# yingqichao/video-watermarking-forgery-detection

Measured on AMD Instinct MI355X. Metric: frames/sec training step (embed->JPEG->decode), 256x256, higher is better.
Workload: dtype bf16; 1 GPU; C2: HiDDeN GAN step enc(4x64)->Jpeg50->dec(7x64)+disc(3x64), L=30, 256x256, batch 16/GPU; not launched (results identical): the generator pass's dead discriminator weight gradients, the decoder's input gradient that Jpeg's zero-gradient rounding multiplies by 0 -- reference_state (--full) times the step with them; global_batch=16, parallelism=dp1

## Files before the change

video_watermarking_forgery_detection_amd/csrc/heads.hip:

```cpp
#include "wm_common.h"

namespace {

template <typename T, int COUT>
__global__ __launch_bounds__(256) void head_fwd_kernel(const T* __restrict__ y, int ldy, const float* __restrict__ scale,
                                                       const float* __restrict__ shift, const float* __restrict__ w,
                                                       const float* __restrict__ bias, float* __restrict__ out, size_t npix,
                                                       size_t hw, int Cin, int act, T* __restrict__ act16) {
    constexpr int VE = vec16<T>::N;
    const int VPP = Cin / VE, PPB = 256 / VPP;
    const int vv = threadIdx.x % VPP, ps = threadIdx.x / VPP;
    const int c0 = vv * VE;
    float sc[VE], sh[VE], wr[COUT][VE];
#pragma unroll
    for (int e = 0; e < VE; ++e) {
        sc[e] = scale ? scale[c0 + e] : 1.f;
        sh[e] = scale ? shift[c0 + e] : 0.f;
#pragma unroll
        for (int co = 0; co < COUT; ++co) wr[co][e] = w[co * Cin + c0 + e];
    }
    constexpr int UN = 4;
    for (size_t base = (size_t)blockIdx.x * PPB * UN; base < npix; base += (size_t)gridDim.x * PPB * UN) {
        vec16<T> yv[UN];
        bool valid[UN];
#pragma unroll
        for (int u = 0; u < UN; ++u) {
            const size_t p = base + (size_t)u * PPB + ps;
            valid[u] = p < npix;
            yv[u] = *reinterpret_cast<const vec16<T>*>(y + (valid[u] ? p : npix - 1) * ldy + c0);
        }
#pragma unroll
        for (int u = 0; u < UN; ++u) {
            const size_t p = base + (size_t)u * PPB + ps;
            float part[COUT];
#pragma unroll
            for (int co = 0; co < COUT; ++co) part[co] = 0.f;
#pragma unroll
            for (int e = 0; e < VE; ++e) {
                float a = sc[e] * yv[u].get(e) + sh[e];
                if (scale) a = fmaxf(a, 0.f);
#pragma unroll
                for (int co = 0; co < COUT; ++co) part[co] += wr[co][e] * a;
            }
            for (int o = VPP >> 1; o > 0; o >>= 1) {
#pragma unroll
                for (int co = 0; co < COUT; ++co) part[co] += __shfl_xor(part[co], o, 64);
            }
            if (valid[u]) {
                for (int oc = vv; oc < COUT; oc += VPP) {
                    float v = 0.f;
#pragma unroll
                    for (int co = 0; co < COUT; ++co) v = (oc == co) ? part[co] + bias[co] : v;
                    if (act == 1) v = 1.f / (1.f + __expf(-v));
                    const size_t b = p / hw, q = p - b * hw;
                    out[(b * COUT + oc) * hw + q] = v;
                }
            }
            if (act16 && valid[u]) {
                for (int pc = vv; pc < 16 / VE; pc += VPP) {
                    vec16<T> o;
#pragma unroll
                    for (int e = 0; e < VE; ++e) {
                        float val = 0.f;
#pragma unroll
                        for (int co = 0; co < COUT; ++co) val = (pc * VE + e == co) ? part[co] + bias[co] : val;
                        o.set(e, val);
                    }
                    *reinterpret_cast<vec16<T>*>(act16 + p * 16 + pc * VE) = o;
                }
            }
        }
    }
}

template <typename T, int COUT>
__global__ __launch_bounds__(256) void head_bwd_kernel(const T* __restrict__ y, int ldy, const float* __restrict__ scale,
                                                       const float* __restrict__ shift, const float* __restrict__ w,
                                                       const float* __restrict__ gout, T* __restrict__ g, int ldg,
                                                       float* __restrict__ partials, size_t npix, size_t hw, int Cin,
                                                       float* __restrict__ bn_partials) {
    constexpr int VE = vec16<T>::N;
    const int VPP = Cin / VE, PPB = 256 / VPP;
    const int vv = threadIdx.x % VPP, ps = threadIdx.x / VPP;
    const int c0 = vv * VE;
    float sc[VE], sh[VE], wr[COUT][VE], dw[COUT][VE], db[COUT];
#pragma unroll
    for (int e = 0; e < VE; ++e) {
        sc[e] = scale ? scale[c0 + e] : 1.f;
        sh[e] = scale ? shift[c0 + e] : 0.f;
#pragma unroll
        for (int co = 0; co < COUT; ++co) { wr[co][e] = w[co * Cin + c0 + e]; dw[co][e] = 0.f; }
    }
#pragma unroll
    for (int co = 0; co < COUT; ++co) db[co] = 0.f;
    float b1[VE], b2[VE];
#pragma unroll
    for (int e = 0; e < VE; ++e) { b1[e] = 0.f; b2[e] = 0.f; }
    for (size_t p = (size_t)blockIdx.x * PPB + ps; p < npix; p += (size_t)gridDim.x * PPB) {
        const size_t b = p / hw, q = p - b * hw;
        float go[COUT];
#pragma unroll
        for (int co = 0; co < COUT; ++co) go[co] = gout[(b * COUT + co) * hw + q];
        const vec16<T> yv = *reinterpret_cast<const vec16<T>*>(y + p * ldy + c0);
        vec16<T> gv;
#pragma unroll
        for (int e = 0; e < VE; ++e) {
            float a = sc[e] * yv.get(e) + sh[e];
            if (scale) a = fmaxf(a, 0.f);
            float gg = 0.f;
#pragma unroll
            for (int co = 0; co < COUT; ++co) { gg += go[co] * wr[co][e]; dw[co][e] += go[co] * a; }
            gv.set(e, gg);
            if (bn_partials) {
                const float gz = a > 0.f ? gv.get(e) : 0.f;
                b1[e] += gz;
                b2[e] = __builtin_fmaf(gz, yv.get(e), b2[e]);
            }
        }
        if (vv == 0) {
#pragma unroll
            for (int co = 0; co < COUT; ++co) db[co] += go[co];
        }
// ... 15 lines not shown
        float s = 0.f;
        for (int qq = 0; qq < PPB; ++qq) s += red[qq * VPP + v2][co * VE + e];
        prow[i] = s;
    }
    if (threadIdx.x < COUT) {
        float s = 0.f;
        for (int qq = 0; qq < PPB; ++qq) s += red[qq * VPP][COUT * VE + threadIdx.x];
        prow[COUT * Cin + threadIdx.x] = s;
    }
    if (bn_partials) {
        __syncthreads();
#pragma unroll
        for (int e = 0; e < VE; ++e) { red[threadIdx.x][e] = b1[e]; red[threadIdx.x][VE + e] = b2[e]; }
        __syncthreads();
        for (int i = threadIdx.x; i < 2 * Cin; i += 256) {
            const int which = i / Cin, c = i - which * Cin;
            const int v2 = c / VE, e = c - v2 * VE;
            float s = 0.f;
            for (int qq = 0; qq < PPB; ++qq) s += red[qq * VPP + v2][which * VE + e];
            bn_partials[((size_t)blockIdx.x * 2 + which) * Cin + c] = s;
        }
    }
}

bool cin_ok(int Cin, int dtype) {
    const int ve = dtype != WM_F32 ? 8 : 4;
    if (Cin <= 0 || Cin % ve) return false;
    const int vpp = Cin / ve;
    return vpp <= 64 && (vpp & (vpp - 1)) == 0;
}

inline int head_parts(size_t npix) {
    const size_t n = (npix + 511) / 512;
    return (int)(n < 1 ? 1 : (n > 1024 ? 1024 : n));
}

}

extern "C" int wm_conv1x1_head_fwd(const void* y, int ldy, const float* scale, const float* shift, const float* w,
                                   const float* bias, float* out, int B, size_t hw, int Cin, int Cout, int act, int dtype,
                                   void* stream) {
    return wm_conv1x1_head_fwd_act(y, ldy, scale, shift, w, bias, out, nullptr, B, hw, Cin, Cout, act, dtype, stream);
}

extern "C" int wm_conv1x1_head_fwd_act(const void* y, int ldy, const float* scale, const float* shift, const float* w,
                                       const float* bias, float* out, void* act16, int B, size_t hw, int Cin, int Cout, int act, int dtype,
                                       void* stream) {
    WM_REQUIRE(y && w && bias && out, WM_E_BADARG, "wm_conv1x1_head_fwd: null pointer");
    WM_REQUIRE(!act16 || (act == 0 && ((uintptr_t)act16 & 15) == 0), WM_E_BADARG, "wm_conv1x1_head_fwd_act: act16 goes with act == 0 and a 16-byte aligned pointer");
    WM_REQUIRE((scale == nullptr) == (shift == nullptr), WM_E_BADARG, "wm_conv1x1_head_fwd: scale/shift must come together");
    WM_REQUIRE(cin_ok(Cin, dtype), WM_E_SHAPE, "wm_conv1x1_head_fwd: unsupported Cin=%d", Cin);
    WM_REQUIRE(Cout == 1 || Cout == 3, WM_E_SHAPE, "wm_conv1x1_head_fwd: Cout must be 1 or 3 (got %d)", Cout);
    const size_t npix = (size_t)B * hw;
    const int grid = (int)((npix + 127) / 128 > 2048 ? 2048 : (npix + 127) / 128);
    hipStream_t s = (hipStream_t)stream;
    WM_DISPATCH_DTYPE(dtype, "wm_conv1x1_head_fwd",
        if (Cout == 3) hipLaunchKernelGGL((head_fwd_kernel<T, 3>), dim3(grid), dim3(256), 0, s, (const T*)y, ldy, scale, shift, w, bias, out, npix, hw, Cin, act, (T*)act16);
        else hipLaunchKernelGGL((head_fwd_kernel<T, 1>), dim3(grid), dim3(256), 0, s, (const T*)y, ldy, scale, shift, w, bias, out, npix, hw, Cin, act, (T*)act16));
    WM_LAUNCH_CHECK("wm_conv1x1_head_fwd");
    return WM_OK;
}

extern "C" int wm_conv1x1_head_nparts(size_t npix) { return head_parts(npix); }

extern "C" int wm_conv1x1_head_bwd(const void* y, int ldy, const float* scale, const float* shift, const float* w,
                                   const float* gout, void* g, int ldg, float* partials, float* bn_partials, int B, size_t hw, int Cin,
                                   int Cout, int dtype, void* stream) {
    WM_REQUIRE(y && w && gout && g && partials, WM_E_BADARG, "wm_conv1x1_head_bwd: null pointer");
    WM_REQUIRE(!bn_partials || scale, WM_E_BADARG, "wm_conv1x1_head_bwd: bn_partials need the producing layer's scale / shift");
    WM_REQUIRE((scale == nullptr) == (shift == nullptr), WM_E_BADARG, "wm_conv1x1_head_bwd: scale/shift must come together");
    WM_REQUIRE(cin_ok(Cin, dtype), WM_E_SHAPE, "wm_conv1x1_head_bwd: unsupported Cin=%d", Cin);
    WM_REQUIRE(Cout == 1 || Cout == 3, WM_E_SHAPE, "wm_conv1x1_head_bwd: Cout must be 1 or 3 (got %d)", Cout);
    const size_t npix = (size_t)B * hw;
    const int grid = head_parts(npix);
    hipStream_t s = (hipStream_t)stream;
    WM_DISPATCH_DTYPE(dtype, "wm_conv1x1_head_bwd",
        if (Cout == 3) hipLaunchKernelGGL((head_bwd_kernel<T, 3>), dim3(grid), dim3(256), 0, s, (const T*)y, ldy, scale, shift, w, gout, (T*)g, ldg, partials, npix, hw, Cin, bn_partials);
        else hipLaunchKernelGGL((head_bwd_kernel<T, 1>), dim3(grid), dim3(256), 0, s, (const T*)y, ldy, scale, shift, w, gout, (T*)g, ldg, partials, npix, hw, Cin, bn_partials));
    WM_LAUNCH_CHECK("wm_conv1x1_head_bwd");
    return WM_OK;
}

namespace {
__global__ __launch_bounds__(256) void linear_head_fwd_kernel(const float* __restrict__ pooled, int ldp, const float* __restrict__ w,
                                                              const float* __restrict__ bias, float* __restrict__ out, int B, int I,
                                                              int O) {
    for (int idx = threadIdx.x; idx < B * O; idx += 256) {
        const int b = idx / O, o = idx - b * O;
        float acc = bias ? bias[o] : 0.f;
        for (int i = 0; i < I; ++i) acc = fmaf(pooled[(size_t)b * ldp + i], w[(size_t)o * I + i], acc);
        out[idx] = acc;
    }
}
__global__ __launch_bounds__(256) void linear_head_bwd_kernel(const float* __restrict__ pooled, int ldp, const float* __restrict__ w,
                                                              const float* __restrict__ g, float* __restrict__ dw,
                                                              float* __restrict__ db, int accumulate, float* __restrict__ gvec,
                                                              int CP, float inv_hw, int B, int I, int O) {
    const int t0 = blockIdx.x * 256 + threadIdx.x, ts = gridDim.x * 256;
    for (int idx = t0; idx < O * I; idx += ts) {
        const int o = idx / I, i = idx - o * I;
        float acc = 0.f;
        for (int b = 0; b < B; ++b) acc = fmaf(g[(size_t)b * O + o], pooled[(size_t)b * ldp + i], acc);
        dw[idx] = (accumulate ? dw[idx] : 0.f) + acc;
    }
    for (int o = t0; o < O; o += ts) {
        float acc = 0.f;
        for (int b = 0; b < B; ++b) acc += g[(size_t)b * O + o];
        db[o] = (accumulate ? db[o] : 0.f) + acc;
    }
    for (int idx = t0; idx < B * CP; idx += ts) {
        const int b = idx / CP, i = idx - b * CP;
// ... 142 lines not shown
```

video_watermarking_forgery_detection_amd/csrc/conv3x3_ws.hip:

```cpp
#include <stdlib.h>
#include "wm_common.h"

#ifdef WM_H16_F16
typedef f16_t hx_t;
#define WM_HSYM(name) name##_f16
#else
typedef bf16_t hx_t;
#define WM_HSYM(name) name##_bf16
#endif
typedef h16<hx_t> HX;
typedef HX::x8 hx8;
typedef HX::x2 hx2;

namespace {

constexpr int TH = 16, TW = 16, HH = 18, HW = 18;
constexpr int C64 = 64;
constexpr int NPIX = HH * HW;

struct WsArgs {
    const hx_t* x; int ldx;
    const hx_t* wp;
    const float* bias; int nbias;
    const float* in_scale; const float* in_shift;
    hx_t* y;
    int ldy;
    float* stat;
    int B, H, W, tilesX, tilesY, ntiles, tiles_per_wg;
    const float* bw_stats4; int bw_ld; const float* bw_coef; const float* bw_gvec;
    const hx_t* ry; const float* r_scale; const float* r_shift;
    const hx_t* ay; hx_t* dy_out;
    int reverse;
    unsigned mX, mY;
};

inline void ws_magic(WsArgs& a) {
    auto m = [](int d) { return d == 1 ? 0u : (unsigned)(((1ull << 32) + (unsigned)d - 1) / (unsigned)d); };
    a.mX = m(a.tilesX); a.mY = m(a.tilesY);
}

template <int CIN> __device__ __forceinline__ int swz(int row, int slot) { return CIN == 64 ? slot ^ ((row >> 1) & 7) : slot; }
template <int CIN> __device__ __forceinline__ int swz_px(int px, int slot) { return CIN == 64 ? slot ^ ((px >> 1) & 7) : slot; }

typedef float f32x2 __attribute__((ext_vector_type(2)));
typedef unsigned u32x4 __attribute__((ext_vector_type(4)));
typedef short i16x2 __attribute__((ext_vector_type(2)));

__device__ __forceinline__ float ws_elu(float z) {
    const float e = __expf(z) - 1.f;
    const float p = z * __builtin_fmaf(z, __builtin_fmaf(z, 0.16666667f, 0.5f), 1.f);
    const float neg = __builtin_fabsf(z) < 0.015625f ? p : e;
    return z > 0.f ? z : neg;
}

template <int CIN, int COUT, bool XFORM, bool STATS, bool M16 = false, int BNBWD = 0, bool BWDST = false, bool ADDIN = false, bool WHOLE = false,
          int ACT = 0, bool NARROW = false>
__global__ __launch_bounds__(512, 2) void conv3x3_ws_kernel(WsArgs a) {
    static_assert(!NARROW || (M16 && COUT == 32 && !BWDST && !ADDIN && !STATS), "NARROW: an input gradient towards a 16-channel (stride) tensor");
    static_assert(ACT == 0 || (!STATS && !BWDST && BNBWD == 0 && !ADDIN), "ACT: plain forward form");
    static_assert(BNBWD != 3 || (!STATS && !BWDST && M16), "BNBWD == 3: no other reduction in the same launch");
    static_assert(!ADDIN || (M16 && !BWDST && BNBWD == 0), "ADDIN: forward form of the 16x16x32 consumers");
    static_assert(CIN == 64 || CIN == 32 || CIN == 16, "input channels");
    static_assert(!M16 || CIN % 32 == 0, "the 16x16x32 MFMA consumes 32 input channels per step");
    static_assert(COUT == 64 || (COUT == 32 && M16), "32 output channels (image dgrads, the 30-channel layer) only with the 16x16x32 consumers");
    constexpr int VPP = CIN / 8;
    constexpr int KS = CIN / 16;
    constexpr int NSTEP = 9 * KS;
    constexpr int XVP = (NPIX * VPP + 255) / 256;
    constexpr int SW_BYTES = 9 * COUT * CIN * 2, SX_BYTES = NPIX * CIN * 2;
    __shared__ __attribute__((aligned(16))) unsigned char smem[SW_BYTES + 2 * SX_BYTES + 4 * 2 * C64 * 4 + C64 * 4];
    hx_t* sW = reinterpret_cast<hx_t*>(smem);
    hx_t* sX0 = reinterpret_cast<hx_t*>(smem + SW_BYTES);
    float* sRed = reinterpret_cast<float*>(smem + SW_BYTES + 2 * SX_BYTES);
    float* sBias = sRed + 4 * 2 * C64;

    const int tid = threadIdx.x, lane = tid & 63, wave = tid >> 6;
    const bool producer = wave >= 4;
    if (tid < COUT) sBias[tid] = (a.bias && tid < a.nbias) ? a.bias[tid] : 0.f;

    constexpr int NV = 9 * COUT * VPP, WV = (NV + 511) / 512;
    hx8 wv[WV];
#pragma unroll
    for (int k = 0; k < WV; ++k) {
        const int i = min(tid + 512 * k, NV - 1);
        wv[k] = *reinterpret_cast<const hx8*>(a.wp + (size_t)(i / VPP) * CIN + (i % VPP) * 8);
    }
    auto commit_filter = [&]() {
#pragma unroll
        for (int k = 0; k < WV; ++k) {
            const int i = tid + 512 * k;
            const int row = i / VPP, tap = row / COUT, n = row % COUT;
            const int c = n & 31, ci = c & 15;
            const int rho = (ci & 3) + 8 * (ci >> 2) + 4 * (c >> 4);
            constexpr int CPL = COUT / 4, NFR = COUT / 16;
            const int lrow = M16 ? tap * COUT + ((n >> 2) % NFR) * 16 + 4 * (n / CPL) + (n & 3) : tap * COUT + (n >> 5) * 32 + rho;
            if (i < NV) *reinterpret_cast<hx8*>(sW + lrow * CIN + swz<CIN>(lrow, i % VPP) * 8) = wv[k];
        }
    };

    const int G = gridDim.x;
    const int run = (G & 7) == 0 ? (blockIdx.x & 7) * (G >> 3) + (blockIdx.x >> 3) : blockIdx.x;
    const int t_begin = run * a.tiles_per_wg;
    const int t_end = min(a.ntiles, t_begin + a.tiles_per_wg);
    struct TileGeo { int b, ty0, tx0; };
    auto fdiv = [](int t, int d, unsigned m) { return d == 1 ? t : (int)__umulhi((unsigned)t, m); };
    auto geo = [&](int tile) {
        TileGeo g;
        const int t = a.reverse ? t_begin + (t_end - 1 - tile) : tile;
        const int q1 = fdiv(t, a.tilesX, a.mX), txi = t - q1 * a.tilesX;
        const int q2 = fdiv(q1, a.tilesY, a.mY), tyi = q1 - q2 * a.tilesY;
        g.b = q2; g.ty0 = tyi * TH; g.tx0 = txi * TW;
        return g;
    };

    if (producer) {
        const int ptid = tid - 256;
        const int vec = ptid % VPP;
        f32x2 sc2[4], sh2[4];
#pragma unroll
        for (int e = 0; e < 4; ++e) { sc2[e] = f32x2{1.f, 1.f}; sh2[e] = f32x2{0.f, 0.f}; }
        if (XFORM) {
#pragma unroll
            for (int e = 0; e < 4; ++e) {
// ... 146 lines not shown
                for (int k = 0; k < XVP; ++k) {
                    u32x4 w = __builtin_bit_cast(u32x4, dG[k]);
                    const u32x4 wy = __builtin_bit_cast(u32x4, dY[k]);
                    const unsigned inimg = (ok >> k) & 1u, keep = 0u - inimg;
                    const float own = (((wmask >> k) & 1u) && inimg) ? 1.f : 0.f;
#pragma unroll
                    for (int pq = 0; pq < 4; ++pq) {
                        float d0, d1;
                        if (BNBWD == 3) {
                            const float o0 = HX::lo(wy[pq]), o1 = HX::hi(wy[pq]);
                            d0 = HX::lo(w[pq]) * (o0 > 0.f ? 1.f : o0 + 1.f);
                            d1 = HX::hi(w[pq]) * (o1 > 0.f ? 1.f : o1 + 1.f);
                            bsum[2 * pq] = __builtin_fmaf(d0, own, bsum[2 * pq]);
                            bsum[2 * pq + 1] = __builtin_fmaf(d1, own, bsum[2 * pq + 1]);
                        } else {
                            d0 = wm_bn_fold_dyg(HX::lo(wy[pq]), HX::lo(w[pq]), kb[0][2 * pq],
                                                kb[1][2 * pq], kca[2 * pq], kb[2][2 * pq], kb[3][2 * pq]);
                            d1 = wm_bn_fold_dyg(HX::hi(wy[pq]), HX::hi(w[pq]),
                                                kb[0][2 * pq + 1], kb[1][2 * pq + 1], kca[2 * pq + 1], kb[2][2 * pq + 1], kb[3][2 * pq + 1]);
                        }
                        const hx2 pk = HX::pack2(d0, d1);
                        w[pq] = __builtin_bit_cast(unsigned, pk);
                    }
#pragma unroll
                    for (int q = 0; q < 4; ++q) w[q] &= keep;
                    if (k + 1 < XVP || last_live) *reinterpret_cast<u32x4*>(sX + lds[k]) = w;
                    if (((wmask >> k) & 1u) && inimg && a.dy_out) *reinterpret_cast<u32x4*>(a.dy_out + tofs + rel[k]) = w;
                }
            };
            if (t_begin < t_end) load_both(geo(t_begin));
            commit_filter();
            if (t_begin < t_end) put_both(sX0, geo(t_begin));
            __syncthreads();
            for (int tile = t_begin; tile < t_end; ++tile) {
                if (tile + 1 < t_end) {
                    const TileGeo g1 = geo(tile + 1);
                    load_both(g1);
                    put_both(sX0 + (((tile - t_begin) & 1) ^ 1) * (NPIX * CIN), g1);
                }
                __syncthreads();
            }
            if (BNBWD == 3) {
#pragma unroll
                for (int e = 0; e < 8; ++e) {
                    float u = bsum[e];
#pragma unroll
                    for (int o = 8; o < 64; o <<= 1) u += __shfl_xor(u, o, 64);
                    if (lane < 8) sRed[(wave - 4) * C64 + vec * 8 + e] = u;
                }
            }
            if (STATS || BWDST || BNBWD == 3) __syncthreads();
            return;
        }
        hx8 dA[XVP], dB[XVP];
        unsigned okA = 0, okB = 0;
        if (t_begin < t_end) load_tile(geo(t_begin), dA, okA, false);
        if (t_begin + 1 < t_end) load_tile(geo(t_begin + 1), dB, okB, reuse_of(t_begin + 1));
        commit_filter();
        if (t_begin < t_end) {
            load_gvec(geo(t_begin).b);
#pragma unroll
            for (int k = 0; k < XVP; ++k) put_one(sX0, k, dA[k], okA);
        }
        __syncthreads();
        auto iter = [&](int tile, hx8 (&nxt)[XVP], unsigned& oknxt, const hx8 (&cur)[XVP], unsigned okcur) {
            hx_t* sXn = sX0 + (((tile - t_begin) & 1) ^ 1) * (NPIX * CIN);
            const hx_t* sXc = sX0 + ((tile - t_begin) & 1) * (NPIX * CIN);
            const bool have_next = tile + 2 < t_end;
            const bool reuse_cur = reuse_of(tile + 1), reuse_nxt = reuse_of(tile + 2);
            if (BNBWD == 1 && tile + 1 < t_end) load_gvec(geo(tile + 1).b);
            if (have_next) {
                const TileGeo g2 = geo(tile + 2);
                if (is_interior(g2)) {
                    const hx_t* xt = tile_ptr(g2);
                    oknxt = 0xffffffffu;
#pragma unroll
                    for (int k = 0; k < KMAIN; ++k) {
                        load_interior(xt, k, nxt[k]);
                        put_one(sXn, k, cur[k], okcur);
                        __builtin_amdgcn_sched_barrier(0);
                    }
                    if (!reuse_nxt) {
#pragma unroll
                        for (int k = KMAIN; k < XVP; ++k) load_interior(xt, k, nxt[k]);
                    }
                } else {
                    const hx_t* xb = image_ptr(g2);
                    oknxt = 0;
#pragma unroll
                    for (int k = 0; k < KMAIN; ++k) {
                        load_border(g2, xb, k, nxt[k], oknxt);
                        put_one(sXn, k, cur[k], okcur);
                        __builtin_amdgcn_sched_barrier(0);
                    }
                    if (!reuse_nxt) {
#pragma unroll
                        for (int k = KMAIN; k < XVP; ++k) load_border(g2, xb, k, nxt[k], oknxt);
                    }
                }
            } else if (tile + 1 < t_end) {
#pragma unroll
                for (int k = 0; k < KMAIN; ++k) put_one(sXn, k, cur[k], okcur);
            }
            if (tile + 1 < t_end) {
                if (reuse_cur) {
#pragma unroll
                    for (int k = KMAIN; k < XVP; ++k) copy_edge(sXn, sXc, k);
                } else {
#pragma unroll
                    for (int k = KMAIN; k < XVP; ++k) put_one(sXn, k, cur[k], okcur);
                }
            }
            __syncthreads();
        };
        for (int tile = t_begin; tile < t_end; tile += 2) {
            iter(tile, dA, okA, dB, okB);
            if (tile + 1 < t_end) iter(tile + 1, dB, okB, dA, okA);
        }
        if (STATS || BWDST) __syncthreads();
        return;
    }

    commit_filter();
    if constexpr (M16) {
        constexpr int KS2 = CIN / 32, NSTEP2 = 9 * KS2;
        constexpr int CPL = COUT / 4;
        constexpr int NFR = COUT / 16;
        constexpr int NPAIR = CPL / 2;
        constexpr int NDR = 2 * (NPAIR + 1);
        const int p = lane & 15, q = lane >> 4;
        float s1[CPL], s2[CPL];
#pragma unroll
        for (int c = 0; c < CPL; ++c) { s1[c] = 0.f; s2[c] = 0.f; }
        int aoff[3][KS2], boff[KS2];
#pragma unroll
        for (int kw = 0; kw < 3; ++kw)
#pragma unroll
            for (int ks = 0; ks < KS2; ++ks)
                aoff[kw][ks] = ((wave * 4 * HW + p + kw) * CIN + swz_px<CIN>(p + kw, ks * 4 + q) * 8) * 2;
#pragma unroll
        for (int ks = 0; ks < KS2; ++ks) boff[ks] = (p * CIN + swz<CIN>(p, ks * 4 + q) * 8) * 2;

        f32x4 acc[4][NFR];
        static_assert(!BWDST || (!STATS && COUT == 64), "BWDST: 64-channel dgrads");
        struct Drain { hx_t* yp; float mk; bool inb; };
        float rsc[CPL], rsh[CPL];
        if (BWDST) {
#pragma unroll
            for (int c = 0; c < CPL; ++c) { rsc[c] = a.r_scale[CPL * q + c]; rsh[c] = a.r_shift[CPL * q + c]; }
        }
        unsigned ryv[2][NPAIR];
        auto load_ry = [&](const Drain (&d)[2]) {
            if (BWDST || ADDIN) {
#pragma unroll
                for (int ml = 0; ml < 2; ++ml) {
                    const hx_t* src = a.ry + (d[ml].inb ? (d[ml].yp - a.y) : (ptrdiff_t)(CPL * q));
#pragma unroll
                    for (int v = 0; v < NPAIR / 4; ++v) {
                        const u32x4 t = *reinterpret_cast<const u32x4*>(src + 8 * v);
                        ryv[ml][4 * v] = t[0]; ryv[ml][4 * v + 1] = t[1]; ryv[ml][4 * v + 2] = t[2]; ryv[ml][4 * v + 3] = t[3];
                    }
                }
            }
        };
        auto drain_of = [&](const TileGeo& g, int mf) {
            Drain d;
            const int gy = g.ty0 + wave * 4 + mf, gx = g.tx0 + p;
            d.inb = WHOLE ? true : (gy < a.H && gx < a.W);
            if (NARROW) d.inb = d.inb && CPL * q < a.ldy;
            d.mk = BWDST ? (d.inb ? 0.f : __builtin_inff()) : (d.inb ? 1.f : 0.f);
            d.yp = a.y + (((size_t)g.b * a.H + gy) * a.W + gx) * (NARROW ? a.ldy : COUT) + CPL * q;
            return d;
// ... 92 lines not shown
                } else {
                    load_ry(d1);
#pragma unroll
                    for (int m = 0; m < NDR; ++m) drain_step(m, 1, d1);
                }
            }
        }
        if (BNBWD == 3) {
            __syncthreads();
            if (tid < C64) a.stat[(size_t)blockIdx.x * C64 + tid] = sRed[tid] + sRed[C64 + tid] + sRed[2 * C64 + tid] + sRed[3 * C64 + tid];
        }
        if (STATS || BWDST) {
            int tid_post = threadIdx.x;
            asm volatile("" : "+v"(tid_post));
            const int q_post = (tid_post & 63) >> 4, wave_post = tid_post >> 6;
#pragma unroll
            for (int c = 0; c < CPL; ++c) {
                float u1 = s1[c], u2 = s2[c];
#pragma unroll
                for (int o = 8; o > 0; o >>= 1) { u1 += __shfl_xor(u1, o, 64); u2 += __shfl_xor(u2, o, 64); }
                if ((tid_post & 15) == 0) {
                    sRed[(wave_post * 2 + 0) * COUT + CPL * q_post + c] = u1;
                    sRed[(wave_post * 2 + 1) * COUT + CPL * q_post + c] = u2;
                }
            }
            __syncthreads();
            if (tid < 2 * COUT) {
                const int which = tid / COUT, n = tid - which * COUT;
                a.stat[((size_t)blockIdx.x * 2 + which) * COUT + n] =
                    sRed[(0 * 2 + which) * COUT + n] + sRed[(1 * 2 + which) * COUT + n] + sRed[(2 * 2 + which) * COUT + n] +
                    sRed[(3 * 2 + which) * COUT + n];
            }
        }
        return;
    }
    const int r = lane & 31, h = lane >> 5;
    f32x2 s1[2][8], s2[2][8];
#pragma unroll
    for (int nf = 0; nf < 2; ++nf)
#pragma unroll
        for (int j = 0; j < 8; ++j) { s1[nf][j] = f32x2{0.f, 0.f}; s2[nf][j] = f32x2{0.f, 0.f}; }
    int aoff[3][KS], boff[KS];
#pragma unroll
    for (int kw = 0; kw < 3; ++kw)
#pragma unroll
        for (int ks = 0; ks < KS; ++ks) {
            const int px = (r & 15) + kw;
            aoff[kw][ks] = (((wave * 4 + (r >> 4)) * HW + px) * CIN + swz_px<CIN>(px, ks * 2 + h) * 8) * 2;
        }
#pragma unroll
    for (int ks = 0; ks < KS; ++ks) boff[ks] = (r * CIN + swz<CIN>(r, ks * 2 + h) * 8) * 2;

    f32x16 acc[2][2];
    struct Drain { hx_t* yp; float mk; bool inb; };
    auto drain_of = [&](const TileGeo& g, int mf) {
        Drain d;
        const int gy = g.ty0 + wave * 4 + mf * 2 + (r >> 4), gx = g.tx0 + (r & 15);
        d.inb = WHOLE ? true : (gy < a.H && gx < a.W);
        d.mk = d.inb ? 1.f : 0.f;
        d.yp = a.y + (((size_t)g.b * a.H + gy) * a.W + gx) * C64 + 16 * h;
        return d;
    };
    unsigned pk[8];
    auto drain_step = [&](int m, int mf, const Drain& d) {
        const int nf = m / 9, j = m - nf * 9;
        if (j < 8) {
            float v0 = acc[mf][nf][2 * j], v1 = acc[mf][nf][2 * j + 1];
            if (ACT == 1) { v0 = ws_elu(v0); v1 = ws_elu(v1); }
            if (STATS) {
                const float t0 = v0 * d.mk, t1 = v1 * d.mk;
                s1[nf][j][0] += t0; s1[nf][j][1] += t1;
                s2[nf][j][0] = __builtin_fmaf(t0, v0, s2[nf][j][0]);
                s2[nf][j][1] = __builtin_fmaf(t1, v1, s2[nf][j][1]);
            }
            const hx2 p2 = HX::pack2(v0, v1);
            pk[j] = __builtin_bit_cast(unsigned, p2);
        } else if (d.inb) {
            *reinterpret_cast<u32x4*>(d.yp + nf * 32) = u32x4{pk[0], pk[1], pk[2], pk[3]};
            *reinterpret_cast<u32x4*>(d.yp + nf * 32 + 8) = u32x4{pk[4], pk[5], pk[6], pk[7]};
        }
    };
    auto pass = [&](const hx_t* sX, int mf, bool drain, int dmf, const Drain& d) {
#pragma unroll
        for (int nf = 0; nf < 2; ++nf) acc[mf][nf] = *reinterpret_cast<const f32x16*>(sBias + nf * 32 + 16 * h);
        constexpr int PF = STATS ? 2 : 3;
        hx8 af[PF], bfr[PF][2];
        auto load_frags = [&](int sidx, int buf) {
            const int tap = sidx / KS, ks = sidx % KS;
            const int kh = tap / 3, kw = tap - kh * 3;
            af[buf] = *reinterpret_cast<const hx8*>(reinterpret_cast<const char*>(sX) + aoff[kw][ks] + (mf * 2 + kh) * (HW * CIN * 2));
#pragma unroll
            for (int nf = 0; nf < 2; ++nf)
                bfr[buf][nf] = *reinterpret_cast<const hx8*>(reinterpret_cast<const char*>(sW) + boff[ks] + (tap * C64 + nf * 32) * (CIN * 2));
        };
#pragma unroll
        for (int i = 0; i < PF - 1; ++i) load_frags(i, i);
#pragma unroll
        for (int sidx = 0; sidx < NSTEP; ++sidx) {
            const int cb = sidx % PF;
            if (sidx + PF - 1 < NSTEP) load_frags(sidx + PF - 1, (sidx + PF - 1) % PF);
            __builtin_amdgcn_sched_barrier(0);
#pragma unroll
            for (int nf = 0; nf < 2; ++nf)
                acc[mf][nf] = HX::mfma32(bfr[cb][nf], af[cb], acc[mf][nf]);
            if (drain) {
#pragma unroll
                for (int m = sidx * 18 / NSTEP; m < (sidx + 1) * 18 / NSTEP; ++m) drain_step(m, dmf, d);
            }
            __builtin_amdgcn_sched_barrier(0);
        }
    };
    __syncthreads();

    if (t_begin < t_end) {
        Drain dnone; dnone.yp = a.y; dnone.mk = 0.f; dnone.inb = false;
        pass(sX0, 0, false, 0, dnone);
        for (int tile = t_begin; tile < t_end; ++tile) {
            const TileGeo g = geo(tile);
            const hx_t* sX = sX0 + ((tile - t_begin) & 1) * (NPIX * CIN);
            pass(sX, 1, true, 0, drain_of(g, 0));
            __syncthreads();
            const Drain d1 = drain_of(g, 1);
            if (tile + 1 < t_end) {
                pass(sX0 + (((tile - t_begin) & 1) ^ 1) * (NPIX * CIN), 0, true, 1, d1);
            } else {
#pragma unroll
                for (int m = 0; m < 18; ++m) drain_step(m, 1, d1);
            }
        }
    }
    if (STATS) {
#pragma unroll
        for (int nf = 0; nf < 2; ++nf)
#pragma unroll
            for (int j = 0; j < 8; ++j)
#pragma unroll
                for (int e = 0; e < 2; ++e) {
                    float u1 = s1[nf][j][e], u2 = s2[nf][j][e];
#pragma unroll
                    for (int o = 16; o > 0; o >>= 1) { u1 += __shfl_xor(u1, o, 64); u2 += __shfl_xor(u2, o, 64); }
                    if (r == 0) {
                        const int c = nf * 32 + 16 * h + 2 * j + e;
                        sRed[(wave * 2 + 0) * C64 + c] = u1;
                        sRed[(wave * 2 + 1) * C64 + c] = u2;
                    }
                }
        __syncthreads();
        if (tid < 2 * C64) {
            const int which = tid / C64, n = tid - which * C64;
            a.stat[((size_t)blockIdx.x * 2 + which) * C64 + n] =
                sRed[(0 * 2 + which) * C64 + n] + sRed[(1 * 2 + which) * C64 + n] + sRed[(2 * 2 + which) * C64 + n] +
                sRed[(3 * 2 + which) * C64 + n];
        }
    }
}

}


#ifndef WM_H16_F16
WM_KNOB(g_ws_variant, wm_debug_ws_variant, 0);
#else
static constexpr int g_ws_variant = 0;
#endif

int WM_HSYM(wm_launch_conv3x3_ws)(const void* x, int ldx, int Cin, int CoutP, const void* wp, const float* bias, int nbias, const float* in_scale,
                           const float* in_shift, void* y, float* stat, int B, int H, int W, int wgs, int tiles_per_wg,
                           hipStream_t s, int reverse, const float* bw_stats4 = nullptr, int bw_ld = 0, const float* bw_coef = nullptr,
                           const float* bw_gvec = nullptr, const void* ry = nullptr, const float* r_scale = nullptr,
                           const float* r_shift = nullptr, const void* ay = nullptr, void* dy_out = nullptr, const void* addend = nullptr,
                           int act = 0, int ldy = 0) {
    WsArgs a;
    a.ldy = ldy > 0 ? ldy : CoutP;
    a.x = (const hx_t*)x; a.ldx = ldx; a.wp = (const hx_t*)wp; a.bias = bias; a.nbias = nbias; a.in_scale = in_scale;
    a.in_shift = in_shift; a.y = (hx_t*)y; a.stat = stat; a.B = B; a.H = H; a.W = W;
// ... 16 lines not shown
            hipLaunchKernelGGL((conv3x3_ws_kernel<64, 32, false, false, true, 3, false, false, false, 0, true>), grid, block, 0, s, a);
        else if (a.ldy != CoutP) return WM_E_SHAPE;
        else if (CoutP == 32) hipLaunchKernelGGL((conv3x3_ws_kernel<64, 32, false, false, true, 3, false>), grid, block, 0, s, a);
        else hipLaunchKernelGGL((conv3x3_ws_kernel<64, 64, false, false, true, 3, false>), grid, block, 0, s, a);
        return WM_OK;
    }
    if (act) {
        if (CoutP != 64 || in_scale || stat || bw_stats4 || ry || addend) return WM_E_SHAPE;
        if (Cin == 64) hipLaunchKernelGGL((conv3x3_ws_kernel<64, 64, false, false, true, 0, false, false, false, 1>), grid, block, 0, s, a);
        else if (Cin == 32) hipLaunchKernelGGL((conv3x3_ws_kernel<32, 64, false, false, true, 0, false, false, false, 1>), grid, block, 0, s, a);
        else if (Cin == 16) hipLaunchKernelGGL((conv3x3_ws_kernel<16, 64, false, false, false, 0, false, false, false, 1>), grid, block, 0, s, a);
        else return WM_E_SHAPE;
        return WM_OK;
    }
    if (ay) {
        if (Cin != 64 || (CoutP != 64 && CoutP != 32) || ldx != 64 || in_scale || !bw_stats4 || !bw_coef || bw_gvec ||
            (ry != nullptr) != (stat != nullptr) || (ry && CoutP != 64))
            return WM_E_SHAPE;
        if (CoutP == 32) hipLaunchKernelGGL((conv3x3_ws_kernel<64, 32, false, false, true, 2, false>), grid, block, 0, s, a);
        else if (ry) hipLaunchKernelGGL((conv3x3_ws_kernel<64, 64, false, false, true, 2, true>), grid, block, 0, s, a);
        else hipLaunchKernelGGL((conv3x3_ws_kernel<64, 64, false, false, true, 2, false>), grid, block, 0, s, a);
        return WM_OK;
    }
    if (ry) {
        if (CoutP != 64 || in_scale || !stat || (Cin != 64 && Cin != 32)) return WM_E_SHAPE;
        if (bw_stats4) {
            if (Cin == 64) hipLaunchKernelGGL((conv3x3_ws_kernel<64, 64, false, false, true, 1, true>), grid, block, 0, s, a);
            else hipLaunchKernelGGL((conv3x3_ws_kernel<32, 64, false, false, true, 1, true>), grid, block, 0, s, a);
        } else {
            if (Cin == 64) hipLaunchKernelGGL((conv3x3_ws_kernel<64, 64, false, false, true, 0, true>), grid, block, 0, s, a);
            else hipLaunchKernelGGL((conv3x3_ws_kernel<32, 64, false, false, true, 0, true>), grid, block, 0, s, a);
        }
        return WM_OK;
    }
    if (bw_stats4) {
        if ((Cin != 64 && Cin != 32) || CoutP != 64 || in_scale || stat) return WM_E_SHAPE;
        if (Cin == 64) hipLaunchKernelGGL((conv3x3_ws_kernel<64, 64, false, false, true, 1>), grid, block, 0, s, a);
        else hipLaunchKernelGGL((conv3x3_ws_kernel<32, 64, false, false, true, 1>), grid, block, 0, s, a);
        return WM_OK;
    }
    const bool xf = in_scale != nullptr, st = stat != nullptr;
#define WM_WS_LAUNCH2(CIN_, COUT_, M16_)                                                                          \
    do {                                                                                                          \
        if (xf && st) hipLaunchKernelGGL((conv3x3_ws_kernel<CIN_, COUT_, true, true, M16_>), grid, block, 0, s, a); \
        else if (xf) hipLaunchKernelGGL((conv3x3_ws_kernel<CIN_, COUT_, true, false, M16_>), grid, block, 0, s, a); \
        else if (st) hipLaunchKernelGGL((conv3x3_ws_kernel<CIN_, COUT_, false, true, M16_>), grid, block, 0, s, a); \
        else hipLaunchKernelGGL((conv3x3_ws_kernel<CIN_, COUT_, false, false, M16_>), grid, block, 0, s, a);      \
    } while (0)
#define WM_WS_LAUNCH(CIN_, M16_) WM_WS_LAUNCH2(CIN_, 64, M16_)
    if (Cin == 64 && CoutP == 64 && xf && st && g_ws_variant == 0 && H % TH == 0 && W % TW == 0) {
        hipLaunchKernelGGL((conv3x3_ws_kernel<64, 64, true, true, true, 0, false, false, true>), grid, block, 0, s, a);
        return WM_OK;
    }
    if (Cin == 16 && CoutP == 64 && !xf && st && g_ws_variant == 0 && H % TH == 0 && W % TW == 0) {
        hipLaunchKernelGGL((conv3x3_ws_kernel<16, 64, false, true, false, 0, false, false, true>), grid, block, 0, s, a);
        return WM_OK;
    }
    if (CoutP == 32) WM_WS_LAUNCH2(64, 32, true);
    else if (Cin == 64 && g_ws_variant != 1) WM_WS_LAUNCH(64, true);
    else if (Cin == 64) WM_WS_LAUNCH(64, false);
    else if (Cin == 32) WM_WS_LAUNCH(32, true);
    else WM_WS_LAUNCH(16, false);
#undef WM_WS_LAUNCH
#undef WM_WS_LAUNCH2
    return WM_OK;
}
```

Baseline: 3031 frames/s.

## Restructure 1x1 head forward so each lane writes one pixel's outputs coalesced

Result: no change. 3034 frames/s, median of 6 (+0.1%).

```diff
diff --git a/video_watermarking_forgery_detection_amd/csrc/heads.hip b/video_watermarking_forgery_detection_amd/csrc/heads.hip
--- a/video_watermarking_forgery_detection_amd/csrc/heads.hip
+++ b/video_watermarking_forgery_detection_amd/csrc/heads.hip
@@ -3,12 +3,47 @@
 namespace {
 
 template <typename T, int COUT>
+__device__ __forceinline__ void head_pixel_sums(const vec16<T>& yv, const float* sc, const float* sh, const float (*wr)[vec16<T>::N], bool relu,
+                                                int VPP, float* part) {
+    constexpr int VE = vec16<T>::N;
+#pragma unroll
+    for (int co = 0; co < COUT; ++co) part[co] = 0.f;
+#pragma unroll
+    for (int e = 0; e < VE; ++e) {
+        float a = sc[e] * yv.get(e) + sh[e];
+        if (relu) a = fmaxf(a, 0.f);
+#pragma unroll
+        for (int co = 0; co < COUT; ++co) part[co] += wr[co][e] * a;
+    }
+    for (int o = VPP >> 1; o > 0; o >>= 1) {
+#pragma unroll
+        for (int co = 0; co < COUT; ++co) part[co] += __shfl_xor(part[co], o, 64);
+    }
+}
+
+template <typename T, int COUT>
+__device__ __forceinline__ void head_store_act16(T* __restrict__ act16, size_t p, int vv, int VPP, const float* part, const float* __restrict__ bias) {
+    constexpr int VE = vec16<T>::N;
+    for (int pc = vv; pc < 16 / VE; pc += VPP) {
+        vec16<T> o;
+#pragma unroll
+        for (int e = 0; e < VE; ++e) {
+            float val = 0.f;
+#pragma unroll
+            for (int co = 0; co < COUT; ++co) val = (pc * VE + e == co) ? part[co] + bias[co] : val;
+            o.set(e, val);
+        }
+        *reinterpret_cast<vec16<T>*>(act16 + p * 16 + pc * VE) = o;
+    }
+}
+
+template <typename T, int COUT, int VPPC>
 __global__ __launch_bounds__(256) void head_fwd_kernel(const T* __restrict__ y, int ldy, const float* __restrict__ scale,
                                                        const float* __restrict__ shift, const float* __restrict__ w,
                                                        const float* __restrict__ bias, float* __restrict__ out, size_t npix,
                                                        size_t hw, int Cin, int act, T* __restrict__ act16) {
     constexpr int VE = vec16<T>::N;
-    const int VPP = Cin / VE, PPB = 256 / VPP;
+    const int VPP = VPPC > 0 ? VPPC : Cin / VE, PPB = 256 / VPP;
     const int vv = threadIdx.x % VPP, ps = threadIdx.x / VPP;
     const int c0 = vv * VE;
     float sc[VE], sh[VE], wr[COUT][VE];
@@ -19,55 +54,67 @@
 #pragma unroll
         for (int co = 0; co < COUT; ++co) wr[co][e] = w[co * Cin + c0 + e];
     }
-    constexpr int UN = 4;
-    for (size_t base = (size_t)blockIdx.x * PPB * UN; base < npix; base += (size_t)gridDim.x * PPB * UN) {
-        vec16<T> yv[UN];
-        bool valid[UN];
-#pragma unroll
-        for (int u = 0; u < UN; ++u) {
-            const size_t p = base + (size_t)u * PPB + ps;
-            valid[u] = p < npix;
-            yv[u] = *reinterpret_cast<const vec16<T>*>(y + (valid[u] ? p : npix - 1) * ldy + c0);
-        }
-#pragma unroll
-        for (int u = 0; u < UN; ++u) {
-            const size_t p = base + (size_t)u * PPB + ps;
-            float part[COUT];
-#pragma unroll
-            for (int co = 0; co < COUT; ++co) part[co] = 0.f;
-#pragma unroll
-            for (int e = 0; e < VE; ++e) {
-                float a = sc[e] * yv[u].get(e) + sh[e];
-                if (scale) a = fmaxf(a, 0.f);
-#pragma unroll
-                for (int co = 0; co < COUT; ++co) part[co] += wr[co][e] * a;
-            }
-            for (int o = VPP >> 1; o > 0; o >>= 1) {
-#pragma unroll
-                for (int co = 0; co < COUT; ++co) part[co] += __shfl_xor(part[co], o, 64);
-            }
-            if (valid[u]) {
-                for (int oc = vv; oc < COUT; oc += VPP) {
-                    float v = 0.f;
-#pragma unroll
-                    for (int co = 0; co < COUT; ++co) v = (oc == co) ? part[co] + bias[co] : v;
+    if constexpr (VPPC > 0) {
+        constexpr int PPW = 64 / VPPC;
+        const int psw = (threadIdx.x & 63) / VPPC;
+        const size_t wave = (size_t)blockIdx.x * 4 + (threadIdx.x >> 6), nwaves = (size_t)gridDim.x * 4;
+        for (size_t base = wave * 64; base < npix; base += nwaves * 64) {
+            vec16<T> yv[VPPC];
+#pragma unroll
+            for (int s = 0; s < VPPC; ++s) {
+                const size_t p = base + (size_t)(s * PPW + psw);
+                yv[s] = *reinterpret_cast<const vec16<T>*>(y + (p < npix ? p : npix - 1) * ldy + c0);
+            }
+            float keep[COUT];
+#pragma unroll
+            for (int co = 0; co < COUT; ++co) keep[co] = 0.f;
+#pragma unroll
+            for (int s = 0; s < VPPC; ++s) {
+                const size_t p = base + (size_t)(s * PPW + psw);
+                float part[COUT];
+                head_pixel_sums<T, COUT>(yv[s], sc, sh, wr, scale != nullptr, VPPC, part);
+#pragma unroll
+                for (int co = 0; co < COUT; ++co) keep[co] = (s == vv) ? part[co] + bias[co] : keep[co];
+                if (act16 && p < npix) head_store_act16<T, COUT>(act16, p, vv, VPPC, part, bias);
+            }
+            const size_t p = base + (size_t)(vv * PPW + psw);
+            if (p < npix) {
+                const size_t b = p / hw, q = p - b * hw;
+#pragma unroll
+                for (int co = 0; co < COUT; ++co) {
+                    float v = keep[co];
                     if (act == 1) v = 1.f / (1.f + __expf(-v));
-                    const size_t b = p / hw, q = p - b * hw;
-                    out[(b * COUT + oc) * hw + q] = v;
+                    out[(b * COUT + co) * hw + q] = v;
                 }
             }
-            if (act16 && valid[u]) {
-                for (int pc = vv; pc < 16 / VE; pc += VPP) {
-                    vec16<T> o;
-#pragma unroll
-                    for (int e = 0; e < VE; ++e) {
-                        float val = 0.f;
-#pragma unroll
-                        for (int co = 0; co < COUT; ++co) val = (pc * VE + e == co) ? part[co] + bias[co] : val;
-                        o.set(e, val);
+        }
+    } else {
+        constexpr int UN = 4;
+        for (size_t base = (size_t)blockIdx.x * PPB * UN; base < npix; base += (size_t)gridDim.x * PPB * UN) {
+            vec16<T> yv[UN];
+            bool valid[UN];
+#pragma unroll
+            for (int u = 0; u < UN; ++u) {
+                const size_t p = base + (size_t)u * PPB + ps;
+                valid[u] = p < npix;
+                yv[u] = *reinterpret_cast<const vec16<T>*>(y + (valid[u] ? p : npix - 1) * ldy + c0);
+            }
+#pragma unroll
+            for (int u = 0; u < UN; ++u) {
+                const size_t p = base + (size_t)u * PPB + ps;
+                float part[COUT];
+                head_pixel_sums<T, COUT>(yv[u], sc, sh, wr, scale != nullptr, VPP, part);
+                if (valid[u]) {
+                    for (int oc = vv; oc < COUT; oc += VPP) {
+                        float v = 0.f;
+#pragma unroll
+                        for (int co = 0; co < COUT; ++co) v = (oc == co) ? part[co] + bias[co] : v;
+                        if (act == 1) v = 1.f / (1.f + __expf(-v));
+                        const size_t b = p / hw, q = p - b * hw;
+                        out[(b * COUT + oc) * hw + q] = v;
                     }
-                    *reinterpret_cast<vec16<T>*>(act16 + p * 16 + pc * VE) = o;
                 }
+                if (act16 && valid[u]) head_store_act16<T, COUT>(act16, p, vv, VPP, part, bias);
             }
         }
     }
@@ -189,11 +236,16 @@
     WM_REQUIRE(cin_ok(Cin, dtype), WM_E_SHAPE, "wm_conv1x1_head_fwd: unsupported Cin=%d", Cin);
     WM_REQUIRE(Cout == 1 || Cout == 3, WM_E_SHAPE, "wm_conv1x1_head_fwd: Cout must be 1 or 3 (got %d)", Cout);
     const size_t npix = (size_t)B * hw;
-    const int grid = (int)((npix + 127) / 128 > 2048 ? 2048 : (npix + 127) / 128);
+    const int ve = dtype != WM_F32 ? 8 : 4, vpp = Cin / ve;
+    const bool w64 = vpp == 4 || vpp == 8;
+    const size_t per = w64 ? 256 : 128;
+    const int grid = (int)((npix + per - 1) / per > 2048 ? 2048 : (npix + per - 1) / per);
     hipStream_t s = (hipStream_t)stream;
+#define WM_HEAD_FWD(CO, VP) hipLaunchKernelGGL((head_fwd_kernel<T, CO, VP>), dim3(grid), dim3(256), 0, s, (const T*)y, ldy, scale, shift, w, bias, out, npix, hw, Cin, act, (T*)act16)
     WM_DISPATCH_DTYPE(dtype, "wm_conv1x1_head_fwd",
-        if (Cout == 3) hipLaunchKernelGGL((head_fwd_kernel<T, 3>), dim3(grid), dim3(256), 0, s, (const T*)y, ldy, scale, shift, w, bias, out, npix, hw, Cin, act, (T*)act16);
-        else hipLaunchKernelGGL((head_fwd_kernel<T, 1>), dim3(grid), dim3(256), 0, s, (const T*)y, ldy, scale, shift, w, bias, out, npix, hw, Cin, act, (T*)act16));
+        if (Cout == 3) { if (vpp == 8) WM_HEAD_FWD(3, 8); else if (vpp == 4) WM_HEAD_FWD(3, 4); else WM_HEAD_FWD(3, 0); }
+        else { if (vpp == 8) WM_HEAD_FWD(1, 8); else if (vpp == 4) WM_HEAD_FWD(1, 4); else WM_HEAD_FWD(1, 0); });
+#undef WM_HEAD_FWD
     WM_LAUNCH_CHECK("wm_conv1x1_head_fwd");
     return WM_OK;
 }
```

## Stage first-layer conv outputs in LDS and store them coalesced from producer waves

Applied to the files above, without the earlier changes.

New measurement: 3130 frames/s before, 3137 frames/s after, median of 3. Within noise of the previous version (+0.2%).

```diff
diff --git a/video_watermarking_forgery_detection_amd/csrc/conv3x3_ws.hip b/video_watermarking_forgery_detection_amd/csrc/conv3x3_ws.hip
--- a/video_watermarking_forgery_detection_amd/csrc/conv3x3_ws.hip
+++ b/video_watermarking_forgery_detection_amd/csrc/conv3x3_ws.hip
@@ -54,8 +54,10 @@
 }
 
 template <int CIN, int COUT, bool XFORM, bool STATS, bool M16 = false, int BNBWD = 0, bool BWDST = false, bool ADDIN = false, bool WHOLE = false,
-          int ACT = 0, bool NARROW = false>
+          int ACT = 0, bool NARROW = false, bool STAGE = false>
 __global__ __launch_bounds__(512, 2) void conv3x3_ws_kernel(WsArgs a) {
+    static_assert(!STAGE || (CIN == 16 && COUT == 64 && !XFORM && STATS && !M16 && BNBWD == 0 && !BWDST && !ADDIN && ACT == 0 && !NARROW),
+                  "STAGE: the image-fed first layers' forward only (the 64-channel forms have no LDS left for an output tile)");
     static_assert(!NARROW || (M16 && COUT == 32 && !BWDST && !ADDIN && !STATS), "NARROW: an input gradient towards a 16-channel (stride) tensor");
     static_assert(ACT == 0 || (!STATS && !BWDST && BNBWD == 0 && !ADDIN), "ACT: plain forward form");
     static_assert(BNBWD != 3 || (!STATS && !BWDST && M16), "BNBWD == 3: no other reduction in the same launch");
@@ -68,7 +70,11 @@
     constexpr int NSTEP = 9 * KS;
     constexpr int XVP = (NPIX * VPP + 255) / 256;
     constexpr int SW_BYTES = 9 * COUT * CIN * 2, SX_BYTES = NPIX * CIN * 2;
-    __shared__ __attribute__((aligned(16))) unsigned char smem[SW_BYTES + 2 * SX_BYTES + 4 * 2 * C64 * 4 + C64 * 4];
+    constexpr int SO_BYTES = TH * TW * C64 * 2;
+    constexpr int SO_OFS = SW_BYTES + 2 * SX_BYTES + 4 * 2 * C64 * 4 + C64 * 4;
+    static_assert(!STAGE || SO_OFS % 128 == 0, "the staged output's slot swizzle is an XOR on offsets from a 128-byte aligned base");
+    __shared__ __attribute__((aligned(16))) unsigned char smem[SO_OFS + (STAGE ? 2 * SO_BYTES : 0)];
+    unsigned char* sOut = smem + SO_OFS;
     hx_t* sW = reinterpret_cast<hx_t*>(smem);
     hx_t* sX0 = reinterpret_cast<hx_t*>(smem + SW_BYTES);
     float* sRed = reinterpret_cast<float*>(smem + SW_BYTES + 2 * SX_BYTES);
@@ -321,6 +327,25 @@
             if (STATS || BWDST || BNBWD == 3) __syncthreads();
             return;
         }
+        const int so_lane = ((wave - 4) * 4 * TW + (lane >> 3)) * (C64 * 2) + (((lane & 7) ^ (lane >> 3)) * 16);
+        auto store_out = [&](int k) {
+            const unsigned char* so = sOut + ((k - t_begin) & 1) * SO_BYTES + so_lane;
+            auto part = [&](int tile, int j0) {
+                const TileGeo g = geo(tile);
+                u32x4 v[4];
+#pragma unroll
+                for (int jj = 0; jj < 4; ++jj) v[jj] = *reinterpret_cast<const u32x4*>(so + (j0 + jj) * (8 * C64 * 2));
+#pragma unroll
+                for (int jj = 0; jj < 4; ++jj) {
+                    const int j = j0 + jj;
+                    const int gy = g.ty0 + (wave - 4) * 4 + (j >> 1), gx = g.tx0 + (j & 1) * 8 + (lane >> 3);
+                    hx_t* dst = a.y + (((size_t)g.b * a.H + gy) * a.W + g.tx0) * C64 + (j & 1) * (8 * C64) + lane * 8;
+                    if (WHOLE || (gy < a.H && gx < a.W)) *reinterpret_cast<u32x4*>(dst) = v[jj];
+                }
+            };
+            if (k < t_end) part(k, 0);
+            if (k > t_begin) part(k - 1, 4);
+        };
         hx8 dA[XVP], dB[XVP];
         unsigned okA = 0, okB = 0;
         if (t_begin < t_end) load_tile(geo(t_begin), dA, okA, false);
@@ -337,6 +362,7 @@
             const hx_t* sXc = sX0 + ((tile - t_begin) & 1) * (NPIX * CIN);
             const bool have_next = tile + 2 < t_end;
             const bool reuse_cur = reuse_of(tile + 1), reuse_nxt = reuse_of(tile + 2);
+            if (STAGE && tile > t_begin) store_out(tile - 1);
             if (BNBWD == 1 && tile + 1 < t_end) load_gvec(geo(tile + 1).b);
             if (have_next) {
                 const TileGeo g2 = geo(tile + 2);
@@ -386,7 +412,9 @@
             iter(tile, dA, okA, dB, okB);
             if (tile + 1 < t_end) iter(tile + 1, dB, okB, dA, okA);
         }
+        if (STAGE && t_begin < t_end) store_out(t_end - 1);
         if (STATS || BWDST) __syncthreads();
+        if (STAGE && t_begin < t_end) store_out(t_end);
         return;
     }
 
@@ -585,13 +613,14 @@
     for (int ks = 0; ks < KS; ++ks) boff[ks] = (r * CIN + swz<CIN>(r, ks * 2 + h) * 8) * 2;
 
     f32x16 acc[2][2];
-    struct Drain { hx_t* yp; float mk; bool inb; };
-    auto drain_of = [&](const TileGeo& g, int mf) {
+    struct Drain { hx_t* yp; float mk; bool inb; int so; };
+    auto drain_of = [&](const TileGeo& g, int mf, int buf) {
         Drain d;
         const int gy = g.ty0 + wave * 4 + mf * 2 + (r >> 4), gx = g.tx0 + (r & 15);
         d.inb = WHOLE ? true : (gy < a.H && gx < a.W);
         d.mk = d.inb ? 1.f : 0.f;
         d.yp = a.y + (((size_t)g.b * a.H + gy) * a.W + gx) * C64 + 16 * h;
+        d.so = buf * SO_BYTES + ((wave * 4 + mf * 2 + (r >> 4)) * TW + (r & 15)) * (C64 * 2) + (((r & 7) ^ (2 * h)) * 16);
         return d;
     };
     unsigned pk[8];
@@ -608,6 +637,9 @@
             }
             const hx2 p2 = HX::pack2(v0, v1);
             pk[j] = __builtin_bit_cast(unsigned, p2);
+        } else if (STAGE) {
+            *reinterpret_cast<u32x4*>(sOut + (d.so ^ (nf * 64))) = u32x4{pk[0], pk[1], pk[2], pk[3]};
+            *reinterpret_cast<u32x4*>(sOut + (d.so ^ (nf * 64 + 16))) = u32x4{pk[4], pk[5], pk[6], pk[7]};
         } else if (d.inb) {
             *reinterpret_cast<u32x4*>(d.yp + nf * 32) = u32x4{pk[0], pk[1], pk[2], pk[3]};
             *reinterpret_cast<u32x4*>(d.yp + nf * 32 + 8) = u32x4{pk[4], pk[5], pk[6], pk[7]};
@@ -646,14 +678,15 @@
     __syncthreads();
 
     if (t_begin < t_end) {
-        Drain dnone; dnone.yp = a.y; dnone.mk = 0.f; dnone.inb = false;
+        Drain dnone; dnone.yp = a.y; dnone.mk = 0.f; dnone.inb = false; dnone.so = 0;
         pass(sX0, 0, false, 0, dnone);
         for (int tile = t_begin; tile < t_end; ++tile) {
             const TileGeo g = geo(tile);
             const hx_t* sX = sX0 + ((tile - t_begin) & 1) * (NPIX * CIN);
-            pass(sX, 1, true, 0, drain_of(g, 0));
+            const int ob = STAGE ? (tile - t_begin) & 1 : 0;
+            pass(sX, 1, true, 0, drain_of(g, 0, ob));
             __syncthreads();
-            const Drain d1 = drain_of(g, 1);
+            const Drain d1 = drain_of(g, 1, ob ^ 1);
             if (tile + 1 < t_end) {
                 pass(sX0 + (((tile - t_begin) & 1) ^ 1) * (NPIX * CIN), 0, true, 1, d1);
             } else {
@@ -776,8 +809,9 @@
         hipLaunchKernelGGL((conv3x3_ws_kernel<64, 64, true, true, true, 0, false, false, true>), grid, block, 0, s, a);
         return WM_OK;
     }
-    if (Cin == 16 && CoutP == 64 && !xf && st && g_ws_variant == 0 && H % TH == 0 && W % TW == 0) {
-        hipLaunchKernelGGL((conv3x3_ws_kernel<16, 64, false, true, false, 0, false, false, true>), grid, block, 0, s, a);
+    if (Cin == 16 && CoutP == 64 && !xf && st && g_ws_variant == 0) {
+        if (H % TH == 0 && W % TW == 0) hipLaunchKernelGGL((conv3x3_ws_kernel<16, 64, false, true, false, 0, false, false, true, 0, false, true>), grid, block, 0, s, a);
+        else hipLaunchKernelGGL((conv3x3_ws_kernel<16, 64, false, true, false, 0, false, false, false, 0, false, true>), grid, block, 0, s, a);
         return WM_OK;
     }
     if (CoutP == 32) WM_WS_LAUNCH2(64, 32, true);
```
